# LuxGraph/Lux

Hardware: NVIDIA H100
Metric: MTEPS (higher is better)
Workload: dtype f32

## Files before the change

include/lux_b200.h:

```cpp
#ifndef LUX_B200_H_
#define LUX_B200_H_

#include <stddef.h>
#include <stdint.h>

#ifdef __cplusplus
extern "C" {
#endif

typedef uint32_t luxb_vid;
typedef uint64_t luxb_eid;

#define LUXB_MAX_PARTS 64
#define LUXB_CF_K 20
#define LUXB_DENSE_BITMAP 0x1234567u
#define LUXB_SPARSE_QUEUE 0x7654321u
#define LUXB_UNIQUE_ID_BYTES 128

typedef enum {
  LUXB_OK = 0,
  LUXB_ERR_ARG = -1,
  LUXB_ERR_CUDA = -2,
  LUXB_ERR_IO = -3,
  LUXB_ERR_COMM = -4,
// ... 85 lines not shown
  uint64_t edges_processed;
  uint64_t pull_iterations;
  uint64_t kernel_launches;
  uint64_t last_active;
  uint32_t last_frontier_type;
  double dominant_kernel_seconds;
  uint64_t dominant_kernel_launches;
  uint64_t panel_edges;
  uint32_t panel_hubs;
  uint32_t panel_blocks;
  uint64_t cold_hub_edges;
  uint32_t cold_hub_segments;
  uint32_t tier_blocks;
  uint64_t tier_slots;
  uint64_t tier_edges;
} luxb_stats_t;
int luxb_stats(const luxb_graph* g, luxb_stats_t* out);
int luxb_trace(const luxb_graph* g, uint64_t* active, int32_t* pull, int max_entries);

int luxb_enable_kernel_timing(luxb_graph* g, int on);
int luxb_get_out_degree(luxb_graph* g, luxb_vid* host_out, size_t bytes);

int luxb_debug_gather_ms(luxb_graph* g, int packed, float* ms_out);

typedef struct {
  void* values;
  const luxb_eid* row_end;
  const luxb_vid* src;
  void* stream;
  luxb_vid row_left, row_right;
// ... 21 lines not shown
```

lux_b200/binding.py:

```python
import ctypes as C
import os
import re
import numpy as np

from . import build as _build

APP_PAGERANK, APP_CC, APP_SSSP, APP_COLFILTER, APP_SSSP_WEIGHTED, APP_BC, APP_BC_WEIGHTED, APP_TC = 0, 1, 2, 3, 4, 5, 6, 7
DIST_INF = 0xFFFFFFFF
EXCHANGE_NCCL, EXCHANGE_P2P, EXCHANGE_P2P_FUSED = 0, 1, 2
DENSE_BITMAP, SPARSE_QUEUE = 0x1234567, 0x7654321
CF_K = 20
MAX_PARTS = 64
UNIQUE_ID_BYTES = 128

_HEADER = os.path.join(os.path.dirname(os.path.abspath(__file__)), "..", "include", "lux_b200.h")
_lib = None


class LuxError(RuntimeError):
    pass


class _Csc(C.Structure):
    _fields_ = [("nv", C.c_uint32), ("ne", C.c_uint64), ("row_end", C.c_void_p), ("src", C.c_void_p),
                ("weight", C.c_void_p)]


class _Config(C.Structure):
    _fields_ = [("app", C.c_int), ("rank", C.c_int), ("nranks", C.c_int), ("device", C.c_int),
                ("start_vtx", C.c_uint32), ("exchange", C.c_int), ("verbose", C.c_int), ("balanced_split", C.c_int),
                ("zero_copy_edges", C.c_int)]


class Stats(C.Structure):
    _fields_ = [("loop_seconds", C.c_double), ("iterations", C.c_uint64), ("edges_processed", C.c_uint64),
                ("pull_iterations", C.c_uint64), ("kernel_launches", C.c_uint64), ("last_active", C.c_uint64),
                ("last_frontier_type", C.c_uint32), ("dominant_kernel_seconds", C.c_double),
                ("dominant_kernel_launches", C.c_uint64), ("panel_edges", C.c_uint64), ("panel_hubs", C.c_uint32),
                ("panel_blocks", C.c_uint32), ("cold_hub_edges", C.c_uint64), ("cold_hub_segments", C.c_uint32),
                ("tier_blocks", C.c_uint32), ("tier_slots", C.c_uint64), ("tier_edges", C.c_uint64)]


class DeviceView(C.Structure):
    _fields_ = [("values", C.c_void_p), ("row_end", C.c_void_p), ("src", C.c_void_p), ("stream", C.c_void_p),
                ("row_left", C.c_uint32), ("row_right", C.c_uint32), ("local_edges", C.c_uint64)]


def library_path():
    return _build.LIB


def declared_symbols():
    text = open(_HEADER).read()
    text = re.sub(r"/\*.*?\*/", "", text, flags=re.S)
    return sorted(set(re.findall(r"\b(luxb_[a-z0-9_]+)\s*\(", text)))


ABI_VERSION = 3


def load_library():
    global _lib
    if _lib is not None:
        return _lib
    path = _build.LIB
    if _build.is_stale():
        try:
            _build.build()
        except Exception as e:
            raise LuxError("libluxb.so is %s and could not be built (%s); lux_b200 has no CPU fallback" % (
                "stale" if os.path.exists(path) else "missing", e))
    L = C.CDLL(path)
    L.luxb_last_error.restype = C.c_char_p
# ... 285 lines not shown
```

lux_b200/csrc/api.cu:

```cuda
#include <cub/cub.cuh>
#include <stdarg.h>
#include <stdlib.h>
#include <string.h>
#include <algorithm>
#include <new>

#include "build.cuh"
#include "cf.cuh"
#include "pull.cuh"
#include "panel.cuh"
#include "seg.cuh"
#include "push.cuh"
#include "runtime.cuh"
#include <thrust/iterator/counting_iterator.h>

using namespace luxb;
static bool is_bc_app(luxb_app app) { return app == LUXB_BC || app == LUXB_BC_WEIGHTED; }
static bool is_tc_app(luxb_app app) { return app == LUXB_TC; }
static bool weighted_labels(luxb_app app) { return app == LUXB_SSSP_WEIGHTED || app == LUXB_BC_WEIGHTED; }
static const char* const kPhaseName[12] = {"pull_tile", "fixup", "refresh", "rechunk", "barrier", "panel", "combine", "pack+push", "pull/bcast", "cold_hub", "bc_sigma", "bc_delta"};
static void pt_mark(luxb_graph* g, int tag) {
  PhaseTimer& pt = g->pt;
  if (!pt.on) return;
  cudaEvent_t e;
// ... 343 lines not shown
    else negative_weight_kernel<<<g->num_sms * 8, 256, 0, g->stream>>>(g->d_weight, g->e_part, d_bad);
    LUXB_CUDA(cudaMemcpyAsync(&neg, d_bad, 8, cudaMemcpyDeviceToHost, g->stream));
    LUXB_CUDA(cudaStreamSynchronize(g->stream));
  }
  LUXB_CUDA(cudaFree(d_tmp));
  LUXB_ARG(bad == 0, "%llu source ids of this rank's slice are >= nv (%u)", bad, g->nv);
  LUXB_ARG(neg == 0 || bc, "%llu edge weights of this rank's slice are negative (weighted SSSP needs w >= 0)", neg);
  LUXB_ARG(neg == 0, "%llu edge weights of this rank's slice are < 1 (weighted betweenness centrality needs w >= 1)", neg);
  return finish_layout(g);
}

extern "C" {

const char* luxb_last_error(void) { return g_err; }
const char* luxb_version(void) { return "lux_b200 0.2 (sm_90a)"; }
int luxb_abi_version(void) { return 3; }

int luxb_partition_csc(luxb_vid nv, luxb_eid ne, const luxb_eid* row_end, int P, luxb_vid* row_left, luxb_vid* row_right,
                       luxb_eid* col_left) {
  LUXB_ARG(row_end && row_left && row_right && col_left, "NULL argument");
  LUXB_ARG(P >= 1 && P <= LUXB_MAX_PARTS, "P out of range");
  LUXB_TRY(validate_row_end(nv, ne, row_end));
  uint32_t np[LUXB_MAX_PARTS];
  int found = host_partition(nv, ne, row_end, P, row_left, np, col_left);
  for (int p = 0; p < P; ++p) row_right[p] = row_left[p] + np[p] - 1;
  return found;
}

int luxb_open_csc(const luxb_csc* csc, const luxb_config* cfg, luxb_graph** out) {
  LUXB_ARG(csc && csc->row_end && (csc->src || csc->ne == 0), "csc arrays are NULL");
  LUXB_TRY(check_config(cfg));
// ... 1086 lines not shown
    blk.ebase[b + 1] = super_end ? blk.ebase[b] + hist[g0 + b] : e_cnt;
  }
  return build_seg_stream<Word, Word>(g, L, d_vrow, n_vtx, d_ids, e_cnt, blk, (uint32_t)shp.stage_edges, (uint32_t)shp.piece, v0, false,
                                      nullptr, super_end);
}
}

static int build_panel_layout(luxb_graph* g) {
  g->sb_on = false;
  g->cs_on = false;
  const SweepSettings& st = g->sweep;
  if (!split_may_run(g) || g->hot_n == 0 || g->e_part == 0 || g->e_part >= 0xFFFFFFFFull) return 0;
  const SegShapeInfo shp = kSegPanelInfo[st.panel_shape];
  const uint32_t bs = st.sb_bs;
  const uint32_t NB0 = (uint32_t)((std::min<uint64_t>(g->hot_n, (uint64_t)st.sb_blocks * bs) + bs - 1) / bs);
  const bool tiers = st.sb_tier > 0 || (st.sb_tier < 0 && g->cold_z && g->e_part >= kSplitMinEdges);
  const uint32_t nb_all = tiers ? (uint32_t)std::min<uint64_t>(((uint64_t)g->hot_n + bs - 1) / bs, kPanelMaxBlocks) : NB0;
  const int grid = g->num_sms * 8;
  DevTmp tmp;

  uint32_t *d_flag = nullptr, *d_hub_idx = nullptr;
  LUXB_TRY(tmp.alloc(&d_flag, (uint64_t)g->n_part + 1));
  LUXB_TRY(tmp.alloc(&d_hub_idx, (uint64_t)g->n_part + 1));
  hub_flag_kernel<<<grid, 256, 0, g->stream>>>(g->d_row_end, g->n_part, st.sb_min_indeg, d_flag);
  LUXB_CUDA(cudaGetLastError());
  LUXB_TRY(cub_call(tmp, g->stream, [&](void* t, size_t& b) {
    return cub::DeviceScan::ExclusiveSum(t, b, d_flag, d_hub_idx, (int)g->n_part, g->stream);
  }));
  uint32_t last_idx = 0, last_flag = 0;
  LUXB_CUDA(cudaMemcpyAsync(&last_idx, d_hub_idx + g->n_part - 1, 4, cudaMemcpyDeviceToHost, g->stream));
  LUXB_CUDA(cudaMemcpyAsync(&last_flag, d_flag + g->n_part - 1, 4, cudaMemcpyDeviceToHost, g->stream));
  LUXB_CUDA(cudaStreamSynchronize(g->stream));
  const uint32_t Nh = last_idx + last_flag;
  if (Nh == 0 || (uint64_t)Nh * NB0 >= 0x7FFFFFF0ull) return 0;
  uint32_t *d_hub_vtx = nullptr, *d_hub_bits = nullptr, *d_cov = nullptr;
  LUXB_TRY(tmp.alloc(&d_hub_vtx, Nh));
  LUXB_TRY(tmp.alloc(&d_hub_bits, ((uint64_t)g->n_part + 31) / 32 + 1));
  LUXB_TRY(tmp.alloc(&d_cov, Nh));
  hub_list_kernel<<<grid, 256, 0, g->stream>>>(d_flag, d_hub_idx, g->n_part, d_hub_vtx, d_hub_bits);
  LUXB_CUDA(cudaGetLastError());
  std::vector<uint32_t> hub_key(Nh);
  {
    uint32_t *d_hkey = nullptr, *d_hkey2 = nullptr, *d_hvtx2 = nullptr;
    LUXB_TRY(tmp.alloc(&d_hkey, Nh));
    LUXB_TRY(tmp.alloc(&d_hkey2, Nh));
    LUXB_TRY(tmp.alloc(&d_hvtx2, Nh));
    hub_order_key_kernel<<<grid, 256, 0, g->stream>>>(g->d_row_end, d_hub_vtx, Nh, d_hkey);
    LUXB_CUDA(cudaGetLastError());
    LUXB_TRY(cub_call(tmp, g->stream, [&](void* t, size_t& b) {
      return cub::DeviceRadixSort::SortPairs(t, b, d_hkey, d_hkey2, d_hub_vtx, d_hvtx2, (int)Nh, 0, 32, g->stream);
    }));
    LUXB_CUDA(cudaMemcpyAsync(d_hub_vtx, d_hvtx2, (size_t)Nh * 4, cudaMemcpyDeviceToDevice, g->stream));
    hub_pos_kernel<<<grid, 256, 0, g->stream>>>(d_hub_vtx, Nh, d_hub_idx);
    LUXB_CUDA(cudaGetLastError());
    LUXB_CUDA(cudaMemcpyAsync(hub_key.data(), d_hkey2, (size_t)Nh * 4, cudaMemcpyDeviceToHost, g->stream));
    LUXB_CUDA(cudaStreamSynchronize(g->stream));
    tmp.release(d_hkey);
    tmp.release(d_hkey2);
    tmp.release(d_hvtx2);
  }
  uint32_t NB = nb_all;
  std::vector<uint32_t> n_pref(NB, Nh);
  uint32_t* d_pref = nullptr;
  LUXB_TRY(tmp.alloc(&d_pref, kPanelMaxBlocks));
  LUXB_CUDA(cudaMemcpyAsync(d_pref, n_pref.data(), (size_t)NB * 4, cudaMemcpyHostToDevice, g->stream));

  ColdSplit cs{};
  cs.hot_n = g->hot_n;
  cs.key0 = NB;
  uint32_t S = 0;
  if (g->cold_z && st.cs != 0 && g->cold_n > 0) {
    const uint32_t s_max = 255 - NB0;
    uint64_t seg = std::max<uint64_t>(1, (uint64_t)(st.cs_seg_mb * 1e6 / 4.0));
    seg = std::min<uint64_t>(std::max<uint64_t>(seg, (g->cold_n + s_max - 1) / s_max), g->cold_n);
    const uint32_t n_seg = (uint32_t)((g->cold_n + seg - 1) / seg);
    if ((uint64_t)Nh * n_seg < 0x7FFFFFF0ull) { cs.seg = (uint32_t)seg; S = n_seg; }
  }

  uint16_t *d_key = nullptr, *d_key2 = nullptr;
  uint64_t *d_pay = nullptr, *d_pay2 = nullptr;
  LUXB_TRY(tmp.alloc(&d_key, g->e_part));
  LUXB_TRY(tmp.alloc(&d_key2, g->e_part));
  LUXB_TRY(tmp.alloc(&d_pay, g->e_part));
  LUXB_TRY(tmp.alloc(&d_pay2, g->e_part));
  constexpr int kBins = kSplitKeyMain + 1;
  unsigned long long* d_hist = nullptr;
  LUXB_TRY(tmp.alloc(&d_hist, kBins));
  unsigned long long hist[kBins];
  auto key_edges = [&]() -> int {
    const uint32_t n_src = (uint32_t)std::min<uint64_t>(g->hot_n, (uint64_t)NB * bs);
    edge_iota_kernel<<<grid, 256, 0, g->stream>>>(d_pay, d_key, g->e_part);
    hub_key_kernel<<<grid, 256, 0, g->stream>>>(g->d_row_end, g->d_src_gather, d_hub_vtx, Nh, n_src, bs, d_pref, NB, d_key, d_pay, d_cov, cs);
    LUXB_CUDA(cudaMemsetAsync(d_hist, 0, kBins * 8, g->stream));
    key_hist_kernel<<<grid, 256, 0, g->stream>>>(d_key, g->e_part, d_hist);
    LUXB_CUDA(cudaGetLastError());
    LUXB_CUDA(cudaMemcpyAsync(hist, d_hist, sizeof(hist), cudaMemcpyDeviceToHost, g->stream));
    LUXB_CUDA(cudaStreamSynchronize(g->stream));
    return 0;
  };
  LUXB_TRY(key_edges());
  bool rekey = false;
  if (tiers && NB > NB0) {
    uint64_t e_hub = 0;
    for (uint32_t h = 0; h < Nh; ++h) e_hub += ~hub_key[h];
    for (uint32_t b = NB0; b < NB; ++b) {
      uint32_t keep = 0;
      if (hist[b] > 0) {
        const double d_min = st.sb_slot_edges * (double)e_hub / (double)hist[b];
        keep = (uint32_t)(std::partition_point(hub_key.begin(), hub_key.end(), [&](uint32_t k) { return (double)~k >= d_min; }) - hub_key.begin());
      }
      n_pref[b] = std::min(keep, n_pref[b - 1]);
      rekey |= n_pref[b] < Nh;
    }
    while (NB > NB0 && n_pref[NB - 1] == 0) --NB;
    cs.key0 = NB;
    LUXB_CUDA(cudaMemcpyAsync(d_pref, n_pref.data(), (size_t)NB * 4, cudaMemcpyHostToDevice, g->stream));
  }
  uint64_t e_cs = 0;
  for (uint32_t s = 0; s < S; ++s) e_cs += hist[nb_all + s];
  if (S && st.cs < 0 && !(e_cs > 0 && (double)e_cs >= kColdSplitMinShare * (double)g->e_part)) {
    rekey |= e_cs > 0;
    cs.seg = 0;
    S = 0;
  }
  if (rekey) LUXB_TRY(key_edges());
  {
    cub::DoubleBuffer<uint16_t> kb(d_key, d_key2);
    cub::DoubleBuffer<uint64_t> pb(d_pay, d_pay2);
    int hbits = 1;
    while ((1ull << hbits) < (uint64_t)Nh) ++hbits;
    LUXB_TRY(cub_call(tmp, g->stream, [&](void* t, size_t& b) {
      return cub::DeviceRadixSort::SortPairs(t, b, pb, kb, (long long)g->e_part, 32, 32 + hbits, g->stream);
    }));
    LUXB_TRY(cub_call(tmp, g->stream, [&](void* t, size_t& b) {
      return cub::DeviceRadixSort::SortPairs(t, b, kb, pb, (long long)g->e_part, 0, kSplitKeyBits, g->stream);
    }));
    tmp.release(kb.Alternate());
    tmp.release(pb.Alternate());
    d_key2 = kb.Current();
    d_pay2 = pb.Current();
  }
  uint64_t e_cov = 0, e_cov0 = 0, e_cold = 0;
  for (uint32_t b = 0; b < NB; ++b) e_cov += hist[b];
  for (uint32_t b = 0; b < NB0; ++b) e_cov0 += hist[b];
  for (uint32_t s = 0; s < S; ++s) e_cold += hist[NB + s];
  const uint64_t e_main = hist[kSplitKeyMain];
  if (e_cov + e_cold + e_main != g->e_part) {
    set_error("panel split lost edges (%llu + %llu + %llu != %llu)", (unsigned long long)e_cov, (unsigned long long)e_cold,
              (unsigned long long)e_main, (unsigned long long)g->e_part);
    return LUXB_ERR_STATE;
  }
  if (e_cov == 0 || (st.sb < 0 && e_cov < g->e_part / 5)) return 0;

  const uint32_t NG = NB + S;
  LUXB_ARG(NG < kSplitKeyMain, "panel: too many source groups");
  uint64_t n_slots = 0;
  g->sb_groups = SplitGroups{};
  for (uint32_t k = 0; k < NG; ++k) {
    n_slots += k < NB ? n_pref[k] : Nh;
    LUXB_ARG(n_slots < 0x7FFFFFF0ull, "panel: too many (group, hub) slots");
    g->sb_groups.vbase[k + 1] = (uint32_t)n_slots;
  }
  LUXB_TRY(build_group_stream<uint16_t>(g, g->sb_panel, d_key2, d_pay2, e_cov, 0, NB, hist, bs, shp, g->sb_super_end));
  if (S)
    LUXB_TRY(build_group_stream<uint32_t>(g, g->sb_cold, d_key2 + e_cov, d_pay2 + e_cov, e_cold, NB, NG, hist, 0,
                                          kSegMainInfo[st.cs_shape], nullptr));

  uint32_t* d_main_src = nullptr;
  uint64_t* d_main_row = nullptr;
  LUXB_TRY(tmp.alloc(&d_main_src, e_main + 8));
  main_fill_kernel<<<grid, 256, 0, g->stream>>>(d_pay2 + e_cov + e_cold, e_main, g->d_src_gather, d_main_src);
  LUXB_TRY(tmp.alloc(&d_main_row, (uint64_t)g->n_part + 4));
  main_indeg_kernel<<<grid, 256, 0, g->stream>>>(g->d_row_end, g->n_part, d_flag, d_hub_idx, d_cov, d_main_row);
  LUXB_CUDA(cudaGetLastError());
  LUXB_TRY(cub_call(tmp, g->stream, [&](void* t, size_t& b) {
    return cub::DeviceScan::InclusiveSum(t, b, d_main_row, d_main_row, (int)g->n_part, g->stream);
  }));
  uint64_t chk = 0;
  LUXB_CUDA(cudaMemcpyAsync(&chk, d_main_row + g->n_part - 1, 8, cudaMemcpyDeviceToHost, g->stream));
  LUXB_CUDA(cudaStreamSynchronize(g->stream));
  if (chk != e_main) { set_error("panel split: offsets do not add up"); return LUXB_ERR_STATE; }
  tmp.release(d_key2);
  tmp.release(d_pay2);
  LUXB_TRY(build_main_stream(g, d_main_row, d_main_src, e_main, d_hub_bits));
  tmp.release(d_main_row);
  tmp.release(d_main_src);

  LUXB_TRY(dmalloc(&g->d_sb_partial, (uint64_t)n_slots + 1));
  LUXB_CUDA(cudaMemsetAsync(g->d_sb_partial, g->cfg.app == LUXB_SSSP || g->cfg.app == LUXB_BC ? 0xFF : 0, ((size_t)n_slots + 1) * 4, g->stream));
  LUXB_CUDA(cudaStreamSynchronize(g->stream));
  g->d_hub_vtx = d_hub_vtx; tmp.keep(d_hub_vtx);
  g->d_hub_bits = d_hub_bits; tmp.keep(d_hub_bits);
  g->sb_n_hub = Nh;
  g->sb_n_blocks = NB;
  g->sb_n_groups = NG;
  g->sb_bs = bs;
  g->sb_on = true;
  g->cs_on = S > 0;
  const uint64_t NV = g->sb_groups.vbase[NB];
  g->stats.panel_edges = e_cov0;
  g->stats.panel_hubs = Nh;
  g->stats.panel_blocks = NB0;
  g->stats.cold_hub_edges = e_cold;
  g->stats.cold_hub_segments = S;
  g->stats.tier_blocks = NB - NB0;
  g->stats.tier_slots = NV - (uint64_t)NB0 * Nh;
  g->stats.tier_edges = e_cov - e_cov0;
  if (g->cfg.verbose)
    printf("[luxb rank %d] source-blocked sweep: %u hub destinations (in-degree >= %u) x %u blocks of %u hot sources, + %u tier blocks "
           "(%llu slots, %llu edges); panel %llu edges (%.1f %%), cold-hub %llu edges (%u segments of %u values), main %llu edges\n",
           g->cfg.rank, Nh, st.sb_min_indeg, NB0, bs, NB - NB0, (unsigned long long)(NV - (uint64_t)NB0 * Nh), (unsigned long long)(e_cov - e_cov0),
           (unsigned long long)e_cov, 100.0 * e_cov / g->e_part, (unsigned long long)e_cold, S, cs.seg, (unsigned long long)e_main);
  return 0;
}

static int build_seg_sweep(luxb_graph* g) {
  g->seg_on = false;
  g->sb_on = false;
  if (!g->sweep.seg) return 0;
  if (g->n_part == 0 || g->cfg.zero_copy_edges || g->e_part >= 0xFFFFFFF0ull) return 0;
  LUXB_TRY(build_panel_layout(g));
  if (!g->sb_on) LUXB_TRY(build_main_stream(g, g->d_row_end, g->hot_n ? g->d_src_gather : g->d_src, g->e_part, nullptr));
  g->seg_on = true;
  return 0;
}

extern "C++" {
// ... 44 lines not shown

extern "C++" {
template <class Prog>
static int launch_seg_main(luxb_graph* g, PullLayout& L, const typename Prog::Vertex* x_nat, const typename Prog::Vertex* x_cold,
                           typename Prog::Vertex* out_local, int out_buffer, const typename Prog::Params& prm, const uint32_t* hub_bits) {
  SegArgs<Prog> a{};
  a.p.n_part = L.n_vtx;
  a.p.row_left = g->row_left;
  a.p.x_nat = x_nat;
  a.p.x_old = x_cold;
  a.p.x_hot = reinterpret_cast<const typename Prog::Vertex*>(g->d_hot);
  a.p.hot_n = g->hot_n;
  a.p.out = out_local;
  a.p.prm = prm;
  a.p.hub_bits = hub_bits;
  a.p.l2_hints = g->l2_hints;
  LUXB_TRY(wait_cold_exchange(g));
  LUXB_TRY((launch_seg_stream<false, Prog>(g, L, a, g->sweep.main_shape, g->pull_ctas, 2, 0, "seg")));
  if (out_buffer >= 0 && L.n_empty && !g->empties_done[out_buffer]) {
    empties_kernel<Prog><<<grid_for(L.n_empty, 256, g->num_sms * 8), 256, 0, g->stream>>>(a.p, L.d_empty, L.n_empty);
    g->empties_done[out_buffer] = true;
    g->stats.kernel_launches++;
  }
  if (L.n_empty_hub) {
    empties_kernel<Prog><<<grid_for(L.n_empty_hub, 256, g->num_sms * 8), 256, 0, g->stream>>>(a.p, L.d_empty_hub, L.n_empty_hub);
    g->stats.kernel_launches++;
  }
  LUXB_CUDA(cudaGetLastError());
  pt_mark(g, 1);
  return 0;
// ... 21 lines not shown
    ca.p.x_old = x_cold;
    ca.p.x_hot = reinterpret_cast<const typename Prog::Vertex*>(g->d_hot);
    ca.p.hot_n = g->hot_n;
    ca.p.out = reinterpret_cast<typename Prog::Vertex*>(g->d_sb_partial);
    ca.p.raw_out = 1;
    ca.p.l2_hints = 0;
    ca.p.prm = prm;
    LUXB_TRY((launch_seg_stream<false, Prog>(g, g->sb_cold, ca, g->sweep.cs_shape, g->pull_ctas, 4, 9, "cold-hub")));
    pt_mark(g, 1);
  }
  LUXB_TRY((launch_seg_main<Prog>(g, g->sb_main, x_nat, x_cold, out_local, out_buffer, prm, g->sb_on ? g->d_hub_bits : nullptr)));
  LUXB_TRY(kt_end(g));
  if (g->sb_on) {
    CombineArgs<Prog> ca{};
    ca.hub_vtx = g->d_hub_vtx;
    ca.n_hub = g->sb_n_hub;
    ca.n_blocks = g->sb_n_blocks;
    ca.n_groups = g->sb_n_groups;
    ca.row_left = g->row_left;
    ca.sg = g->sb_groups;
    ca.partial = reinterpret_cast<const Acc*>(g->d_sb_partial);
    ca.x_nat = x_nat;
    ca.out = out_local;
    ca.prm = prm;
    combine_hub_kernel<Prog><<<grid_for(g->sb_n_hub, 256, g->num_sms * 8), 256, 0, g->stream>>>(ca);
    LUXB_CUDA(cudaGetLastError());
    g->stats.kernel_launches++;
    pt_mark(g, 6);
  }
  return 0;
}
}

static int pagerank_publish(luxb_graph* g, float* x_new) {
  const int me = g->cfg.rank;
  const int grid = g->num_sms * 8;
  if (g->P == 1 || !g->packed) {
    if (g->P > 1) { LUXB_TRY(allgather_slices(g, x_new, 4)); pt_mark(g, 3); }
    if (g->hot_n) {
// ... 1115 lines not shown
                  g->d_out_w, g->d_fq_all, g->d_fq_new, g->d_fq_tmp, g->d_hdr_all, g->d_counters, g->d_chunk_first, g->d_chunk_vtx,
                  g->d_partial, g->d_sync, g->d_hot_order, g->d_src_gather, g->d_hot, g->d_big_list, g->d_sigma, g->d_delta,
                  g->d_scores, g->d_order, g->d_bc_lvl, g->d_bc_off, g->d_bc_split, g->d_bc_sort_tmp, g->d_bc_ctl, g->d_bc_hubs,
                  g->d_bc_partial, g->d_tc_off, g->d_tc_dst, g->d_tc_staged, g->d_tc_stage_pre, g->d_tc_group, g->d_tc_big,
                  g->d_tc_t, g->d_tc_total, g->d_tc_next, g->d_tc_sum_tmp};
  for (void* p : ptrs) {
    if (!p) continue;
    if (std::find(g->host_allocs.begin(), g->host_allocs.end(), p) != g->host_allocs.end()) cudaFreeHost(p);
    else cudaFree(p);
  }
  free_layout(g->base, false);
  free_layout(g->sb_main);
  free_layout(g->sb_panel);
  free_layout(g->sb_cold);
  if (g->d_hub_vtx) cudaFree(g->d_hub_vtx);
  if (g->d_hub_bits) cudaFree(g->d_hub_bits);
  if (g->d_sb_partial) cudaFree(g->d_sb_partial);
  for (void* q : {(void*)g->d_zperm, (void*)g->d_pack_list, (void*)g->d_xt[0], (void*)g->d_xt[1], (void*)g->d_fctl, (void*)g->d_slot_off, (void*)g->d_flags})
    if (q) cudaFree(q);
  if (g->h_barrier_err) cudaFreeHost(g->h_barrier_err);
  if (g->h_hdr) cudaFreeHost(g->h_hdr);
  if (g->h_scratch) cudaFreeHost(g->h_scratch);
  for (cudaEvent_t e : g->kt_events) cudaEventDestroy(e);
  if (g->ev_begin) cudaEventDestroy(g->ev_begin);
  if (g->ev_end) cudaEventDestroy(g->ev_end);
  if (g->stream) cudaStreamDestroy(g->stream);
  delete g;
}

}
```

lux_b200/csrc/panel.cuh:

```cuda
#pragma once
#include "common.cuh"
#include "programs.cuh"
#include "pull.cuh"

namespace luxb {

constexpr int kPanelMaxBlocks = 256;
constexpr uint16_t kSplitKeyMain = 511;
constexpr int kSplitKeyBits = 9;

struct SplitGroups {
  uint32_t vbase[kSplitKeyMain + 1];
};

__global__ void hub_flag_kernel(const uint64_t* __restrict__ row_end_rel, uint32_t n_part, uint32_t min_indeg,
                                uint32_t* __restrict__ flag) {
  for (uint64_t i = (uint64_t)blockIdx.x * blockDim.x + threadIdx.x; i < n_part; i += (uint64_t)gridDim.x * blockDim.x) {
    uint64_t d = row_end_rel[i] - (i == 0 ? 0 : row_end_rel[i - 1]);
    flag[i] = d >= min_indeg ? 1u : 0u;
  }
}

__global__ void hub_list_kernel(const uint32_t* __restrict__ flag, const uint32_t* __restrict__ hub_idx, uint32_t n_part,
                                uint32_t* __restrict__ hub_vtx, uint32_t* __restrict__ hub_bits) {
// ... 22 lines not shown
__global__ void edge_iota_kernel(uint64_t* __restrict__ payload, uint16_t* __restrict__ key, uint64_t n) {
  for (uint64_t e = (uint64_t)blockIdx.x * blockDim.x + threadIdx.x; e < n; e += (uint64_t)gridDim.x * blockDim.x) {
    payload[e] = e;
    key[e] = kSplitKeyMain;
  }
}

struct ColdSplit {
  uint32_t hot_n;
  uint32_t seg;
  uint32_t key0;
};

__global__ void hub_key_kernel(const uint64_t* __restrict__ row_end_rel, const uint32_t* __restrict__ src_gather,
                               const uint32_t* __restrict__ hub_vtx, uint32_t n_hub, uint32_t n_src, uint32_t bs,
                               const uint32_t* __restrict__ n_pref, uint32_t n_blocks,
                               uint16_t* __restrict__ key, uint64_t* __restrict__ payload, uint32_t* __restrict__ cov_count,
                               const ColdSplit cs) {
  __shared__ uint32_t s_pref[kPanelMaxBlocks];
  for (uint32_t i = threadIdx.x; i < n_blocks; i += blockDim.x) s_pref[i] = n_pref[i];
  __syncthreads();
  const unsigned lane = threadIdx.x & 31;
  const uint64_t warps_total = ((uint64_t)gridDim.x * blockDim.x) >> 5;
  for (uint64_t h = ((uint64_t)blockIdx.x * blockDim.x + threadIdx.x) >> 5; h < n_hub; h += warps_total) {
    const uint32_t v = hub_vtx[h];
    const uint64_t b = v == 0 ? 0 : row_end_rel[v - 1], e = row_end_rel[v];
    uint32_t cnt = 0;
    for (uint64_t k = b + lane; k < e; k += 32) {
      const uint32_t id = src_gather[k];
      if (id < n_src) {
        if (h < s_pref[id / bs]) {
          key[k] = (uint16_t)(id / bs);
          payload[k] = (h << 32) | k;
          ++cnt;
        }
      } else if (cs.seg != 0 && id >= cs.hot_n) {
        key[k] = (uint16_t)(cs.key0 + (id - cs.hot_n) / cs.seg);
        payload[k] = (h << 32) | k;
        ++cnt;
      }
    }
#pragma unroll
    for (int off = 16; off; off >>= 1) cnt += __shfl_xor_sync(0xffffffffu, cnt, off);
    if (lane == 0) cov_count[h] = cnt;
  }
}

__global__ void key_hist_kernel(const uint16_t* __restrict__ key, uint64_t n, unsigned long long* __restrict__ hist) {
  constexpr int kBins = kSplitKeyMain + 1;
  __shared__ unsigned int s_h[kBins];
  for (int i = threadIdx.x; i < kBins; i += blockDim.x) s_h[i] = 0;
  __syncthreads();
  for (uint64_t e = (uint64_t)blockIdx.x * blockDim.x + threadIdx.x; e < n; e += (uint64_t)gridDim.x * blockDim.x)
    atomicAdd(&s_h[key[e]], 1u);
  __syncthreads();
  for (int i = threadIdx.x; i < kBins; i += blockDim.x)
    if (s_h[i]) atomicAdd(hist + i, (unsigned long long)s_h[i]);
}

// ... 17 lines not shown
}

__global__ void main_indeg_kernel(const uint64_t* __restrict__ row_end_rel, uint32_t n_part, const uint32_t* __restrict__ flag,
                                  const uint32_t* __restrict__ hub_idx, const uint32_t* __restrict__ cov_count,
                                  uint64_t* __restrict__ out) {
  for (uint64_t i = (uint64_t)blockIdx.x * blockDim.x + threadIdx.x; i < n_part; i += (uint64_t)gridDim.x * blockDim.x) {
    uint64_t d = row_end_rel[i] - (i == 0 ? 0 : row_end_rel[i - 1]);
    if (flag[i]) d -= cov_count[hub_idx[i]];
    out[i] = d;
  }
}

template <class Prog>
struct CombineArgs {
  const uint32_t* hub_vtx;
  uint32_t n_hub, n_blocks, n_groups, row_left;
  SplitGroups sg;
  const typename Prog::Acc* partial;
  const typename Prog::Vertex* x_nat;
  typename Prog::Vertex* out;
  typename Prog::Params prm;
};

template <class Prog>
__global__ void combine_hub_kernel(const __grid_constant__ CombineArgs<Prog> a) {
  for (uint64_t h = (uint64_t)blockIdx.x * blockDim.x + threadIdx.x; h < a.n_hub; h += (uint64_t)gridDim.x * blockDim.x) {
    const uint32_t v = a.hub_vtx[h];
    typename Prog::Acc raw0;
    memcpy(&raw0, &a.out[v], sizeof(raw0));
    typename Prog::Wide t = Prog::widen(raw0);
    uint32_t b = 0;
    for (; b + 8 <= a.n_blocks && h < a.sg.vbase[b + 8] - a.sg.vbase[b + 7]; b += 8) {
      typename Prog::Acc p[8];
#pragma unroll
      for (int i = 0; i < 8; ++i) p[i] = a.partial[a.sg.vbase[b + i] + h];
#pragma unroll
      for (int i = 0; i < 8; ++i) t = Prog::wcombine(t, Prog::widen(p[i]));
    }
    for (; b < a.n_blocks && h < a.sg.vbase[b + 1] - a.sg.vbase[b]; ++b)
      t = Prog::wcombine(t, Prog::widen(a.partial[a.sg.vbase[b] + h]));
    for (uint32_t k = a.n_blocks; k < a.n_groups; ++k) t = Prog::wcombine(t, Prog::widen(a.partial[a.sg.vbase[k] + h]));
    const typename Prog::Vertex oldv = Prog::kNeedsOld ? a.x_nat[a.row_left + v] : typename Prog::Vertex();
    const typename Prog::Vertex nv_ = Prog::update(a.row_left + v, Prog::narrow(t), oldv, a.prm);
    a.out[v] = nv_;
  }
}

}
```

lux_b200/csrc/pull.cuh:

```cuda
#pragma once
#include "common.cuh"
#include "programs.cuh"

namespace luxb {

template <int kIPT_, int kWarps_, int kStages_>
struct PullShape {
  static constexpr int kIPT = kIPT_;
  static constexpr int kWarps = kWarps_;
  static constexpr int kThreads = 32 * (kWarps + 1);
  static constexpr int kTile = 32 * kIPT;
  static constexpr int kSuper = kTile * kWarps;
  static constexpr int kStages = kStages_;
  static constexpr int kAElems = kSuper + 8;
  static constexpr int kEElems = kSuper + 8;
  static constexpr int kSumElems = kTile + 4;
  static constexpr int kHdrElems = kWarps + 4;
  static constexpr size_t kSmemBytes = (size_t)kStages * (kAElems + kEElems) * 4 + (size_t)kWarps * kSumElems * 4 +
                                       2 * kStages * 8 + (size_t)kStages * kHdrElems * 4 + 16;
  static_assert(kIPT % 2 == 1, "kIPT must be odd: lane-contiguous smem reads are then bank-conflict free");
  static constexpr size_t kWRingOffset = (kSmemBytes + 15) & ~(size_t)15;
};

template <class Prog, class Shape>
// ... 20 lines not shown
  uint32_t row_left;
  const typename Prog::Vertex* x_old;
  const typename Prog::Vertex* x_hot;
  uint32_t hot_n;
  const typename Prog::Vertex* x_nat;
  typename Prog::Vertex* out;
  typename Prog::Acc* head_partial;
  typename Prog::Acc* tail_partial;
  typename Prog::Wide* carry;
  uint32_t* carry_flag;
  typename Prog::Wide* block_agg;
  uint32_t* block_flag;
  uint32_t* tile_counter;
  typename Prog::Params prm;
  const uint32_t* hub_bits;
  int raw_out;
  int l2_hints;
  const uint32_t* close_vtx;
};

template <class Prog>
__device__ __forceinline__ bool store_raw(const PullArgs<Prog>& a, uint32_t v) {
  if (a.raw_out) return true;
  return a.hub_bits != nullptr && ((__ldg(a.hub_bits + (v >> 5)) >> (v & 31)) & 1u);
}

template <class Prog>
__device__ __forceinline__ void store_vertex(const PullArgs<Prog>& a, uint32_t v, typename Prog::Acc sum) {
  using Vertex = typename Prog::Vertex;
  if (store_raw(a, v)) {
    Vertex r;
    static_assert(sizeof(Vertex) == sizeof(typename Prog::Acc), "raw sums travel in the value slot");
    memcpy(&r, &sum, sizeof(r));
    a.out[v] = r;
    return;
  }
  Vertex oldv = Prog::kNeedsOld ? __ldg(a.x_nat + a.row_left + v) : Vertex();
  Vertex nv_ = Prog::update(a.row_left + v, sum, oldv, a.prm);
  a.out[v] = nv_;
}

__global__ void tile_table_kernel(const uint64_t* __restrict__ row_end, uint32_t n_part, uint64_t e_part, uint32_t tile,
                                  uint32_t n_tiles, uint32_t* __restrict__ tile_v) {
  uint32_t t = blockIdx.x * blockDim.x + threadIdx.x;
  if (t > n_tiles) return;
  uint64_t total = (uint64_t)n_part + e_part;
  uint64_t d = (uint64_t)t * tile;
  if (d > total) d = total;
  uint64_t lo = d > e_part ? d - e_part : 0, hi = d < n_part ? d : n_part;
  while (lo < hi) {
// ... 459 lines not shown
```

lux_b200/csrc/runtime.cuh:

```cuda
#pragma once
#include <vector>
#include "comm.h"
#include "common.cuh"
#include "panel.cuh"
#include "seg.cuh"
#include "push.cuh"
#include "bc.cuh"
#include "tc.cuh"

struct FixupScratch {
  void* d_head = nullptr;
  void* d_tail = nullptr;
  void* d_carry = nullptr;
  uint32_t* d_carry_flag = nullptr;
  void* d_block_agg = nullptr;
  uint32_t* d_block_flag = nullptr;
  uint32_t n_fix_blocks = 0;
  unsigned long long* d_chain = nullptr;
  uint32_t chain_epoch = 0;
};

struct PullLayout {
  uint64_t* d_row_end = nullptr;
  uint32_t* d_row_end32 = nullptr;
// ... 153 lines not shown
  uint32_t* h_barrier_err = nullptr;
  uint64_t barrier_timeout_ns = 30000000000ull;
  bool flag_barrier = true;
  bool flag_barrier_all = false;
  bool direct_push = false;

  SweepSettings sweep;

  bool empties_done[2] = {false, false};
  bool seg_on = false;
  bool sb_on = false;
  PullLayout sb_main, sb_panel;
  uint32_t sb_n_hub = 0, sb_n_blocks = 0, sb_n_groups = 0, sb_bs = 0;
  uint32_t* d_hub_vtx = nullptr;
  uint32_t* d_hub_bits = nullptr;
  uint32_t* d_sb_partial = nullptr;
  luxb::SplitGroups sb_groups{};
  uint32_t sb_super_end[luxb::kPanelMaxBlocks]{};
  bool cold_z = false;
  bool cs_on = false;
  PullLayout sb_cold;

  int pull_ctas = 3;
  bool overlap_exchange = true;
  bool fused_fixup = true;
  int panel_reserve_sms = 12;
  int l2_hints = 1;
  PhaseTimer pt;

  bool kernel_timing = false;
// ... 10 lines not shown
```

Measured before the change: 172,800.

## Apply per-group hub slot pruning and compact hub raw sums into dense array

Extends the hub-keep rule to all panel blocks and cold-hub segments, dropping hubs no group keeps. Hub raw sums from the main pull go to a compact rank-indexed buffer rather than scattered into the output array. The combine kernel reads it with a per-hub degree array. This aims to cut panel slot count, partial-buffer traffic and scattered accesses during combine, at the cost of extra setup kernels and a popcount rank lookup in the store path.

```diff
diff --git a/include/lux_b200.h b/include/lux_b200.h
--- a/include/lux_b200.h
+++ b/include/lux_b200.h
@@ -123,6 +123,7 @@
   uint32_t tier_blocks;
   uint64_t tier_slots;
   uint64_t tier_edges;
+  uint64_t panel_slots;
 } luxb_stats_t;
 int luxb_stats(const luxb_graph* g, luxb_stats_t* out);
 int luxb_trace(const luxb_graph* g, uint64_t* active, int32_t* pull, int max_entries);
diff --git a/lux_b200/binding.py b/lux_b200/binding.py
--- a/lux_b200/binding.py
+++ b/lux_b200/binding.py
@@ -38,7 +38,8 @@
                 ("last_frontier_type", C.c_uint32), ("dominant_kernel_seconds", C.c_double),
                 ("dominant_kernel_launches", C.c_uint64), ("panel_edges", C.c_uint64), ("panel_hubs", C.c_uint32),
                 ("panel_blocks", C.c_uint32), ("cold_hub_edges", C.c_uint64), ("cold_hub_segments", C.c_uint32),
-                ("tier_blocks", C.c_uint32), ("tier_slots", C.c_uint64), ("tier_edges", C.c_uint64)]
+                ("tier_blocks", C.c_uint32), ("tier_slots", C.c_uint64), ("tier_edges", C.c_uint64),
+                ("panel_slots", C.c_uint64)]
 
 
 class DeviceView(C.Structure):
@@ -56,7 +57,7 @@
     return sorted(set(re.findall(r"\b(luxb_[a-z0-9_]+)\s*\(", text)))
 
 
-ABI_VERSION = 3
+ABI_VERSION = 4
 
 
 def load_library():
diff --git a/lux_b200/csrc/api.cu b/lux_b200/csrc/api.cu
--- a/lux_b200/csrc/api.cu
+++ b/lux_b200/csrc/api.cu
@@ -4,6 +4,7 @@
 #include <string.h>
 #include <algorithm>
 #include <new>
+#include <type_traits>
 
 #include "build.cuh"
 #include "cf.cuh"
@@ -381,7 +382,7 @@
 
 const char* luxb_last_error(void) { return g_err; }
 const char* luxb_version(void) { return "lux_b200 0.2 (sm_90a)"; }
-int luxb_abi_version(void) { return 3; }
+int luxb_abi_version(void) { return 4; }
 
 int luxb_partition_csc(luxb_vid nv, luxb_eid ne, const luxb_eid* row_end, int P, luxb_vid* row_left, luxb_vid* row_right,
                        luxb_eid* col_left) {
@@ -1498,8 +1499,8 @@
   const SegShapeInfo shp = kSegPanelInfo[st.panel_shape];
   const uint32_t bs = st.sb_bs;
   const uint32_t NB0 = (uint32_t)((std::min<uint64_t>(g->hot_n, (uint64_t)st.sb_blocks * bs) + bs - 1) / bs);
-  const bool tiers = st.sb_tier > 0 || (st.sb_tier < 0 && g->cold_z && g->e_part >= kSplitMinEdges);
-  const uint32_t nb_all = tiers ? (uint32_t)std::min<uint64_t>(((uint64_t)g->hot_n + bs - 1) / bs, kPanelMaxBlocks) : NB0;
+  const bool slot_rule = st.sb_tier > 0 || (st.sb_tier < 0 && g->cold_z && g->e_part >= kSplitMinEdges);
+  const uint32_t nb_all = slot_rule ? (uint32_t)std::min<uint64_t>(((uint64_t)g->hot_n + bs - 1) / bs, kPanelMaxBlocks) : NB0;
   const int grid = g->num_sms * 8;
   DevTmp tmp;
 
@@ -1515,7 +1516,7 @@
   LUXB_CUDA(cudaMemcpyAsync(&last_idx, d_hub_idx + g->n_part - 1, 4, cudaMemcpyDeviceToHost, g->stream));
   LUXB_CUDA(cudaMemcpyAsync(&last_flag, d_flag + g->n_part - 1, 4, cudaMemcpyDeviceToHost, g->stream));
   LUXB_CUDA(cudaStreamSynchronize(g->stream));
-  const uint32_t Nh = last_idx + last_flag;
+  uint32_t Nh = last_idx + last_flag;
   if (Nh == 0 || (uint64_t)Nh * NB0 >= 0x7FFFFFF0ull) return 0;
   uint32_t *d_hub_vtx = nullptr, *d_hub_bits = nullptr, *d_cov = nullptr;
   LUXB_TRY(tmp.alloc(&d_hub_vtx, Nh));
@@ -1544,10 +1545,9 @@
     tmp.release(d_hvtx2);
   }
   uint32_t NB = nb_all;
-  std::vector<uint32_t> n_pref(NB, Nh);
+  std::vector<uint32_t> n_pref(kSplitKeyMain, Nh);
   uint32_t* d_pref = nullptr;
-  LUXB_TRY(tmp.alloc(&d_pref, kPanelMaxBlocks));
-  LUXB_CUDA(cudaMemcpyAsync(d_pref, n_pref.data(), (size_t)NB * 4, cudaMemcpyHostToDevice, g->stream));
+  LUXB_TRY(tmp.alloc(&d_pref, kSplitKeyMain));
 
   ColdSplit cs{};
   cs.hot_n = g->hot_n;
@@ -1573,8 +1573,9 @@
   unsigned long long hist[kBins];
   auto key_edges = [&]() -> int {
     const uint32_t n_src = (uint32_t)std::min<uint64_t>(g->hot_n, (uint64_t)NB * bs);
+    LUXB_CUDA(cudaMemcpyAsync(d_pref, n_pref.data(), (size_t)(NB + S) * 4, cudaMemcpyHostToDevice, g->stream));
     edge_iota_kernel<<<grid, 256, 0, g->stream>>>(d_pay, d_key, g->e_part);
-    hub_key_kernel<<<grid, 256, 0, g->stream>>>(g->d_row_end, g->d_src_gather, d_hub_vtx, Nh, n_src, bs, d_pref, NB, d_key, d_pay, d_cov, cs);
+    hub_key_kernel<<<grid, 256, 0, g->stream>>>(g->d_row_end, g->d_src_gather, d_hub_vtx, Nh, n_src, bs, d_pref, NB + S, d_key, d_pay, d_cov, cs);
     LUXB_CUDA(cudaMemsetAsync(d_hist, 0, kBins * 8, g->stream));
     key_hist_kernel<<<grid, 256, 0, g->stream>>>(d_key, g->e_part, d_hist);
     LUXB_CUDA(cudaGetLastError());
@@ -1584,28 +1585,37 @@
   };
   LUXB_TRY(key_edges());
   bool rekey = false;
-  if (tiers && NB > NB0) {
-    uint64_t e_hub = 0;
-    for (uint32_t h = 0; h < Nh; ++h) e_hub += ~hub_key[h];
-    for (uint32_t b = NB0; b < NB; ++b) {
-      uint32_t keep = 0;
-      if (hist[b] > 0) {
-        const double d_min = st.sb_slot_edges * (double)e_hub / (double)hist[b];
-        keep = (uint32_t)(std::partition_point(hub_key.begin(), hub_key.end(), [&](uint32_t k) { return (double)~k >= d_min; }) - hub_key.begin());
-      }
-      n_pref[b] = std::min(keep, n_pref[b - 1]);
-      rekey |= n_pref[b] < Nh;
-    }
-    while (NB > NB0 && n_pref[NB - 1] == 0) --NB;
-    cs.key0 = NB;
-    LUXB_CUDA(cudaMemcpyAsync(d_pref, n_pref.data(), (size_t)NB * 4, cudaMemcpyHostToDevice, g->stream));
-  }
   uint64_t e_cs = 0;
   for (uint32_t s = 0; s < S; ++s) e_cs += hist[nb_all + s];
   if (S && st.cs < 0 && !(e_cs > 0 && (double)e_cs >= kColdSplitMinShare * (double)g->e_part)) {
     rekey |= e_cs > 0;
     cs.seg = 0;
     S = 0;
+  }
+  if (slot_rule) {
+    uint64_t e_hub = 0;
+    for (uint32_t h = 0; h < Nh; ++h) e_hub += ~hub_key[h];
+    auto keep = [&](unsigned long long m) -> uint32_t {
+      if (m == 0) return 0;
+      const double d_min = st.sb_slot_edges * (double)e_hub / (double)m;
+      return (uint32_t)(std::partition_point(hub_key.begin(), hub_key.end(), [&](uint32_t k) { return (double)~k >= d_min; }) - hub_key.begin());
+    };
+    for (uint32_t b = 0; b < NB; ++b) n_pref[b] = std::min(keep(hist[b]), b ? n_pref[b - 1] : Nh);
+    while (NB > 0 && n_pref[NB - 1] == 0) --NB;
+    for (uint32_t s = 0; s < S; ++s) n_pref[NB + s] = keep(hist[nb_all + s]);
+    cs.key0 = NB;
+    uint32_t n_live = 0;
+    for (uint32_t k = 0; k < NB + S; ++k) {
+      n_live = std::max(n_live, n_pref[k]);
+      rekey |= n_pref[k] < Nh;
+    }
+    if (n_live == 0) return 0;
+    if (n_live < Nh) {
+      hub_drop_kernel<<<grid_for(Nh - n_live, 256, grid), 256, 0, g->stream>>>(d_hub_vtx, n_live, Nh, d_flag, d_hub_bits);
+      LUXB_CUDA(cudaGetLastError());
+      Nh = n_live;
+      hub_key.resize(Nh);
+    }
   }
   if (rekey) LUXB_TRY(key_edges());
   {
@@ -1624,10 +1634,12 @@
     d_key2 = kb.Current();
     d_pay2 = pb.Current();
   }
+  const uint32_t nb_first = std::min(NB, NB0);
   uint64_t e_cov = 0, e_cov0 = 0, e_cold = 0;
   for (uint32_t b = 0; b < NB; ++b) e_cov += hist[b];
-  for (uint32_t b = 0; b < NB0; ++b) e_cov0 += hist[b];
+  for (uint32_t b = 0; b < nb_first; ++b) e_cov0 += hist[b];
   for (uint32_t s = 0; s < S; ++s) e_cold += hist[NB + s];
+  if (e_cold == 0) S = 0;
   const uint64_t e_main = hist[kSplitKeyMain];
   if (e_cov + e_cold + e_main != g->e_part) {
     set_error("panel split lost edges (%llu + %llu + %llu != %llu)", (unsigned long long)e_cov, (unsigned long long)e_cold,
@@ -1641,7 +1653,7 @@
   uint64_t n_slots = 0;
   g->sb_groups = SplitGroups{};
   for (uint32_t k = 0; k < NG; ++k) {
-    n_slots += k < NB ? n_pref[k] : Nh;
+    n_slots += n_pref[k];
     LUXB_ARG(n_slots < 0x7FFFFFF0ull, "panel: too many (group, hub) slots");
     g->sb_groups.vbase[k + 1] = (uint32_t)n_slots;
   }
@@ -1669,6 +1681,27 @@
   LUXB_TRY(build_main_stream(g, d_main_row, d_main_src, e_main, d_hub_bits));
   tmp.release(d_main_row);
   tmp.release(d_main_src);
+
+  const uint32_t n_words = (uint32_t)(((uint64_t)g->n_part + 31) / 32);
+  uint32_t* d_wcnt = nullptr;
+  LUXB_TRY(tmp.alloc(&d_wcnt, (uint64_t)n_words + 1));
+  LUXB_TRY(dmalloc(&g->d_hub_base, (uint64_t)n_words + 1));
+  LUXB_TRY(dmalloc(&g->d_hub_rank, (uint64_t)Nh + 1));
+  LUXB_TRY(dmalloc(&g->d_hub_raw, (uint64_t)Nh + 1));
+  const bool hub_deg = g->cfg.app == LUXB_PAGERANK && g->d_deg != nullptr;
+  if (hub_deg) LUXB_TRY(dmalloc(&g->d_hub_deg, (uint64_t)Nh + 1));
+  hub_word_count_kernel<<<grid, 256, 0, g->stream>>>(d_hub_bits, n_words, d_wcnt);
+  LUXB_CUDA(cudaMemsetAsync(d_wcnt + n_words, 0, 4, g->stream));
+  LUXB_TRY(cub_call(tmp, g->stream, [&](void* t, size_t& b) {
+    return cub::DeviceScan::ExclusiveSum(t, b, d_wcnt, g->d_hub_base, (int)n_words + 1, g->stream);
+  }));
+  hub_rank_kernel<<<grid, 256, 0, g->stream>>>(d_hub_vtx, Nh, d_hub_bits, g->d_hub_base, hub_deg ? g->d_deg : nullptr, g->row_left,
+                                               g->d_hub_rank, g->d_hub_deg);
+  LUXB_CUDA(cudaGetLastError());
+  uint32_t n_ranked = 0;
+  LUXB_CUDA(cudaMemcpyAsync(&n_ranked, g->d_hub_base + n_words, 4, cudaMemcpyDeviceToHost, g->stream));
+  LUXB_CUDA(cudaStreamSynchronize(g->stream));
+  if (n_ranked != Nh) { set_error("panel split: %u hub bits for %u hubs", n_ranked, Nh); return LUXB_ERR_STATE; }
 
   LUXB_TRY(dmalloc(&g->d_sb_partial, (uint64_t)n_slots + 1));
   LUXB_CUDA(cudaMemsetAsync(g->d_sb_partial, g->cfg.app == LUXB_SSSP || g->cfg.app == LUXB_BC ? 0xFF : 0, ((size_t)n_slots + 1) * 4, g->stream));
@@ -1681,20 +1714,23 @@
   g->sb_bs = bs;
   g->sb_on = true;
   g->cs_on = S > 0;
-  const uint64_t NV = g->sb_groups.vbase[NB];
+  const uint64_t tier_slots = g->sb_groups.vbase[NB] - g->sb_groups.vbase[nb_first];
   g->stats.panel_edges = e_cov0;
   g->stats.panel_hubs = Nh;
   g->stats.panel_blocks = NB0;
+  g->stats.panel_slots = n_slots;
   g->stats.cold_hub_edges = e_cold;
   g->stats.cold_hub_segments = S;
-  g->stats.tier_blocks = NB - NB0;
-  g->stats.tier_slots = NV - (uint64_t)NB0 * Nh;
+  g->stats.tier_blocks = NB - nb_first;
+  g->stats.tier_slots = tier_slots;
   g->stats.tier_edges = e_cov - e_cov0;
   if (g->cfg.verbose)
-    printf("[luxb rank %d] source-blocked sweep: %u hub destinations (in-degree >= %u) x %u blocks of %u hot sources, + %u tier blocks "
-           "(%llu slots, %llu edges); panel %llu edges (%.1f %%), cold-hub %llu edges (%u segments of %u values), main %llu edges\n",
-           g->cfg.rank, Nh, st.sb_min_indeg, NB0, bs, NB - NB0, (unsigned long long)(NV - (uint64_t)NB0 * Nh), (unsigned long long)(e_cov - e_cov0),
-           (unsigned long long)e_cov, 100.0 * e_cov / g->e_part, (unsigned long long)e_cold, S, cs.seg, (unsigned long long)e_main);
+    printf("[luxb rank %d] source-blocked sweep: %u hub destinations (in-degree >= %u) x %u blocks of %u hot sources (%llu slots), + %u "
+           "blocks (%llu slots, %llu edges); panel %llu edges (%.1f %%), cold-hub %llu edges (%u segments of %u values, %llu slots), main %llu "
+           "edges\n",
+           g->cfg.rank, Nh, st.sb_min_indeg, nb_first, bs, (unsigned long long)g->sb_groups.vbase[nb_first], NB - nb_first,
+           (unsigned long long)tier_slots, (unsigned long long)(e_cov - e_cov0), (unsigned long long)e_cov, 100.0 * e_cov / g->e_part,
+           (unsigned long long)e_cold, S, cs.seg, (unsigned long long)(n_slots - g->sb_groups.vbase[NB]), (unsigned long long)e_main);
   return 0;
 }
 
@@ -1769,6 +1805,8 @@
   a.p.out = out_local;
   a.p.prm = prm;
   a.p.hub_bits = hub_bits;
+  a.p.hub_base = g->d_hub_base;
+  a.p.hub_raw = reinterpret_cast<typename Prog::Acc*>(g->d_hub_raw);
   a.p.l2_hints = g->l2_hints;
   LUXB_TRY(wait_cold_exchange(g));
   LUXB_TRY((launch_seg_stream<false, Prog>(g, L, a, g->sweep.main_shape, g->pull_ctas, 2, 0, "seg")));
@@ -1820,6 +1858,8 @@
   if (g->sb_on) {
     CombineArgs<Prog> ca{};
     ca.hub_vtx = g->d_hub_vtx;
+    ca.hub_rank = g->d_hub_rank;
+    ca.hub_raw = reinterpret_cast<const Acc*>(g->d_hub_raw);
     ca.n_hub = g->sb_n_hub;
     ca.n_blocks = g->sb_n_blocks;
     ca.n_groups = g->sb_n_groups;
@@ -1829,6 +1869,7 @@
     ca.x_nat = x_nat;
     ca.out = out_local;
     ca.prm = prm;
+    if constexpr (std::is_same<Prog, PageRankProgram>::value) ca.prm.deg = g->d_hub_deg;
     combine_hub_kernel<Prog><<<grid_for(g->sb_n_hub, 256, g->num_sms * 8), 256, 0, g->stream>>>(ca);
     LUXB_CUDA(cudaGetLastError());
     g->stats.kernel_launches++;
@@ -2974,7 +3015,7 @@
   free_layout(g->sb_panel);
   free_layout(g->sb_cold);
   if (g->d_hub_vtx) cudaFree(g->d_hub_vtx);
-  if (g->d_hub_bits) cudaFree(g->d_hub_bits);
+  for (uint32_t* q : {g->d_hub_bits, g->d_hub_base, g->d_hub_rank, g->d_hub_raw, g->d_hub_deg}) if (q) cudaFree(q);
   if (g->d_sb_partial) cudaFree(g->d_sb_partial);
   for (void* q : {(void*)g->d_zperm, (void*)g->d_pack_list, (void*)g->d_xt[0], (void*)g->d_xt[1], (void*)g->d_fctl, (void*)g->d_slot_off, (void*)g->d_flags})
     if (q) cudaFree(q);
diff --git a/lux_b200/csrc/panel.cuh b/lux_b200/csrc/panel.cuh
--- a/lux_b200/csrc/panel.cuh
+++ b/lux_b200/csrc/panel.cuh
@@ -60,11 +60,11 @@
 
 __global__ void hub_key_kernel(const uint64_t* __restrict__ row_end_rel, const uint32_t* __restrict__ src_gather,
                                const uint32_t* __restrict__ hub_vtx, uint32_t n_hub, uint32_t n_src, uint32_t bs,
-                               const uint32_t* __restrict__ n_pref, uint32_t n_blocks,
+                               const uint32_t* __restrict__ n_pref, uint32_t n_groups,
                                uint16_t* __restrict__ key, uint64_t* __restrict__ payload, uint32_t* __restrict__ cov_count,
                                const ColdSplit cs) {
-  __shared__ uint32_t s_pref[kPanelMaxBlocks];
-  for (uint32_t i = threadIdx.x; i < n_blocks; i += blockDim.x) s_pref[i] = n_pref[i];
+  __shared__ uint32_t s_pref[kSplitKeyMain];
+  for (uint32_t i = threadIdx.x; i < n_groups; i += blockDim.x) s_pref[i] = n_pref[i];
   __syncthreads();
   const unsigned lane = threadIdx.x & 31;
   const uint64_t warps_total = ((uint64_t)gridDim.x * blockDim.x) >> 5;
@@ -81,14 +81,41 @@
           ++cnt;
         }
       } else if (cs.seg != 0 && id >= cs.hot_n) {
-        key[k] = (uint16_t)(cs.key0 + (id - cs.hot_n) / cs.seg);
-        payload[k] = (h << 32) | k;
-        ++cnt;
+        const uint32_t g = cs.key0 + (id - cs.hot_n) / cs.seg;
+        if (h < s_pref[g]) {
+          key[k] = (uint16_t)g;
+          payload[k] = (h << 32) | k;
+          ++cnt;
+        }
       }
     }
 #pragma unroll
     for (int off = 16; off; off >>= 1) cnt += __shfl_xor_sync(0xffffffffu, cnt, off);
     if (lane == 0) cov_count[h] = cnt;
+  }
+}
+
+__global__ void hub_drop_kernel(const uint32_t* __restrict__ hub_vtx, uint32_t from, uint32_t to, uint32_t* __restrict__ flag,
+                                uint32_t* __restrict__ hub_bits) {
+  for (uint64_t h = from + (uint64_t)blockIdx.x * blockDim.x + threadIdx.x; h < to; h += (uint64_t)gridDim.x * blockDim.x) {
+    const uint32_t v = hub_vtx[h];
+    flag[v] = 0;
+    atomicAnd(&hub_bits[v >> 5], ~(1u << (v & 31)));
+  }
+}
+
+__global__ void hub_word_count_kernel(const uint32_t* __restrict__ hub_bits, uint32_t n_words, uint32_t* __restrict__ cnt) {
+  for (uint64_t w = (uint64_t)blockIdx.x * blockDim.x + threadIdx.x; w < n_words; w += (uint64_t)gridDim.x * blockDim.x)
+    cnt[w] = __popc(hub_bits[w]);
+}
+
+__global__ void hub_rank_kernel(const uint32_t* __restrict__ hub_vtx, uint32_t n_hub, const uint32_t* __restrict__ hub_bits,
+                                const uint32_t* __restrict__ hub_base, const uint32_t* __restrict__ deg, uint32_t row_left,
+                                uint32_t* __restrict__ rank, uint32_t* __restrict__ hub_deg) {
+  for (uint64_t h = (uint64_t)blockIdx.x * blockDim.x + threadIdx.x; h < n_hub; h += (uint64_t)gridDim.x * blockDim.x) {
+    const uint32_t v = hub_vtx[h];
+    rank[h] = hub_base[v >> 5] + __popc(hub_bits[v >> 5] & ((1u << (v & 31)) - 1u));
+    if (deg) hub_deg[h] = deg[row_left + v];
   }
 }
 
@@ -136,6 +163,8 @@
 template <class Prog>
 struct CombineArgs {
   const uint32_t* hub_vtx;
+  const uint32_t* hub_rank;
+  const typename Prog::Acc* hub_raw;
   uint32_t n_hub, n_blocks, n_groups, row_left;
   SplitGroups sg;
   const typename Prog::Acc* partial;
@@ -148,9 +177,7 @@
 __global__ void combine_hub_kernel(const __grid_constant__ CombineArgs<Prog> a) {
   for (uint64_t h = (uint64_t)blockIdx.x * blockDim.x + threadIdx.x; h < a.n_hub; h += (uint64_t)gridDim.x * blockDim.x) {
     const uint32_t v = a.hub_vtx[h];
-    typename Prog::Acc raw0;
-    memcpy(&raw0, &a.out[v], sizeof(raw0));
-    typename Prog::Wide t = Prog::widen(raw0);
+    typename Prog::Wide t = Prog::widen(a.hub_raw[a.hub_rank[h]]);
     uint32_t b = 0;
     for (; b + 8 <= a.n_blocks && h < a.sg.vbase[b + 8] - a.sg.vbase[b + 7]; b += 8) {
       typename Prog::Acc p[8];
@@ -161,9 +188,10 @@
     }
     for (; b < a.n_blocks && h < a.sg.vbase[b + 1] - a.sg.vbase[b]; ++b)
       t = Prog::wcombine(t, Prog::widen(a.partial[a.sg.vbase[b] + h]));
-    for (uint32_t k = a.n_blocks; k < a.n_groups; ++k) t = Prog::wcombine(t, Prog::widen(a.partial[a.sg.vbase[k] + h]));
+    for (uint32_t k = a.n_blocks; k < a.n_groups; ++k)
+      if (h < a.sg.vbase[k + 1] - a.sg.vbase[k]) t = Prog::wcombine(t, Prog::widen(a.partial[a.sg.vbase[k] + h]));
     const typename Prog::Vertex oldv = Prog::kNeedsOld ? a.x_nat[a.row_left + v] : typename Prog::Vertex();
-    const typename Prog::Vertex nv_ = Prog::update(a.row_left + v, Prog::narrow(t), oldv, a.prm);
+    const typename Prog::Vertex nv_ = Prog::update((uint32_t)h, Prog::narrow(t), oldv, a.prm);
     a.out[v] = nv_;
   }
 }
diff --git a/lux_b200/csrc/pull.cuh b/lux_b200/csrc/pull.cuh
--- a/lux_b200/csrc/pull.cuh
+++ b/lux_b200/csrc/pull.cuh
@@ -58,26 +58,29 @@
   uint32_t* tile_counter;
   typename Prog::Params prm;
   const uint32_t* hub_bits;
+  const uint32_t* hub_base;
+  typename Prog::Acc* hub_raw;
   int raw_out;
   int l2_hints;
   const uint32_t* close_vtx;
 };
 
 template <class Prog>
-__device__ __forceinline__ bool store_raw(const PullArgs<Prog>& a, uint32_t v) {
-  if (a.raw_out) return true;
-  return a.hub_bits != nullptr && ((__ldg(a.hub_bits + (v >> 5)) >> (v & 31)) & 1u);
-}
-
-template <class Prog>
 __device__ __forceinline__ void store_vertex(const PullArgs<Prog>& a, uint32_t v, typename Prog::Acc sum) {
   using Vertex = typename Prog::Vertex;
-  if (store_raw(a, v)) {
+  if (a.raw_out) {
     Vertex r;
     static_assert(sizeof(Vertex) == sizeof(typename Prog::Acc), "raw sums travel in the value slot");
     memcpy(&r, &sum, sizeof(r));
     a.out[v] = r;
     return;
+  }
+  if (a.hub_bits != nullptr) {
+    const uint32_t bits = __ldg(a.hub_bits + (v >> 5)), bit = 1u << (v & 31);
+    if (bits & bit) {
+      a.hub_raw[__ldg(a.hub_base + (v >> 5)) + __popc(bits & (bit - 1u))] = sum;
+      return;
+    }
   }
   Vertex oldv = Prog::kNeedsOld ? __ldg(a.x_nat + a.row_left + v) : Vertex();
   Vertex nv_ = Prog::update(a.row_left + v, sum, oldv, a.prm);
diff --git a/lux_b200/csrc/runtime.cuh b/lux_b200/csrc/runtime.cuh
--- a/lux_b200/csrc/runtime.cuh
+++ b/lux_b200/csrc/runtime.cuh
@@ -191,6 +191,10 @@
   uint32_t sb_n_hub = 0, sb_n_blocks = 0, sb_n_groups = 0, sb_bs = 0;
   uint32_t* d_hub_vtx = nullptr;
   uint32_t* d_hub_bits = nullptr;
+  uint32_t* d_hub_base = nullptr;
+  uint32_t* d_hub_rank = nullptr;
+  uint32_t* d_hub_raw = nullptr;
+  uint32_t* d_hub_deg = nullptr;
   uint32_t* d_sb_partial = nullptr;
   luxb::SplitGroups sb_groups{};
   uint32_t sb_super_end[luxb::kPanelMaxBlocks]{};
```

After: 175,900, median of 6. +1.8%, better.
